# NTT123/vietTTS

Hardware: NVIDIA H100
Metric: audio_samples_per_sec (higher is better)
Workload: dtype f32 (bf16x3 split products on wgmma tensor cores, fp32 accumulate/storage)

## Files before the change

### viettts_b200/csrc/api.cu

```cuda
#include <stdarg.h>

#include <algorithm>

#include <dlfcn.h>

#include "stream_common.cuh"

std::string g_vtts_create_error;

int vtts_ctx::fail(int code, const char* fmt, ...) {
  char buf[1024];
  va_list ap;
  va_start(ap, fmt);
  vsnprintf(buf, sizeof(buf), fmt, ap);
  va_end(ap);
  err = buf;
  return code;
}

int vtts_ctx::ensure_ws(size_t bytes) {
  vtts_ctx* ctx = this;
  if (bytes <= ws_bytes) return VTTS_OK;
  clear_taps();
  if (ws) {
// ... 253 lines not shown
int vtts_create(int device, vtts_ctx** out) {
  if (!out) {
    g_vtts_create_error = "vtts_create: out is NULL";
    return VTTS_ERR_BAD_ARG;
  }
  *out = nullptr;
  int n = 0;
  cudaError_t e = cudaGetDeviceCount(&n);
  if (e != cudaSuccess || n == 0) {
    g_vtts_create_error = std::string("vtts_create: no CUDA device (") + cudaGetErrorString(e) + "); there is no CPU fallback";
    cudaGetLastError();
    return VTTS_ERR_NO_DEVICE;
  }
  if (device < 0 || device >= n) {
    g_vtts_create_error = "vtts_create: device index out of range";
    return VTTS_ERR_BAD_ARG;
  }
  cudaDeviceProp prop;
  if ((e = cudaSetDevice(device)) != cudaSuccess || (e = cudaGetDeviceProperties(&prop, device)) != cudaSuccess) {
    g_vtts_create_error = std::string("vtts_create: ") + cudaGetErrorString(e);
    return VTTS_ERR_CUDA;
  }
  if (prop.major != 9 || prop.minor != 0) {
    char buf[256];
    snprintf(buf, sizeof(buf), "vtts_create: device %d is sm_%d%d; this library contains sm_90a code only", device, prop.major, prop.minor);
    g_vtts_create_error = buf;
    return VTTS_ERR_NO_DEVICE;
  }
  vtts_ctx* ctx = new vtts_ctx();
  ctx->device = device;
  ctx->sm_count = prop.multiProcessorCount;
  ctx->cc_major = prop.major;
  ctx->cc_minor = prop.minor;
  ctx->hbm_bytes = prop.totalGlobalMem;
  if ((e = cudaStreamCreateWithFlags(&ctx->own_stream, cudaStreamNonBlocking)) != cudaSuccess) {
    g_vtts_create_error = std::string("vtts_create: ") + cudaGetErrorString(e);
    delete ctx;
    return VTTS_ERR_CUDA;
  }
  for (int i = 0; i < vtts_ctx::NSTAGE; ++i) {
    cudaEventCreate(&ctx->ev0[i]);
    cudaEventCreate(&ctx->ev1[i]);
  }
  if ((e = cudaEventCreateWithFlags(&ctx->tail, cudaEventDisableTiming)) != cudaSuccess) {
    g_vtts_create_error = std::string("vtts_create: ") + cudaGetErrorString(e);
    delete ctx;
    return VTTS_ERR_CUDA;
  }
  if (cudaMalloc(&ctx->d_err, sizeof(int)) != cudaSuccess || cudaMemset(ctx->d_err, 0, sizeof(int)) != cudaSuccess) {
    g_vtts_create_error = "vtts_create: cannot allocate the error flag";
    delete ctx;
    return VTTS_ERR_CUDA;
  }
  if (cudaMalloc(&ctx->d_tc_sched, 2 * sizeof(int)) != cudaSuccess || cudaMemset(ctx->d_tc_sched, 0, 2 * sizeof(int)) != cudaSuccess) {
    g_vtts_create_error = "vtts_create: cannot allocate the tile scheduler counters";
    delete ctx;
    return VTTS_ERR_CUDA;
  }
  if (cudaMalloc(&ctx->d_tc_dbg, 256 * 16 * sizeof(long long)) != cudaSuccess) {
    g_vtts_create_error = "vtts_create: cannot allocate the profiling counters";
    delete ctx;
    return VTTS_ERR_CUDA;
  }
  cudaMemset(ctx->d_tc_dbg, 0, 256 * 16 * sizeof(long long));
  *out = ctx;
  return VTTS_OK;
}

int vtts_destroy(vtts_ctx* ctx) {
  if (!ctx) return VTTS_OK;
  cudaSetDevice(ctx->device);
  cudaDeviceSynchronize();
  for (auto& m : kModels) vtts_free_weights(ctx->*m.w);
  vtts_resample_free(ctx);
  cudaFree(ctx->mel_fb); cudaFree(ctx->mel_lo); cudaFree(ctx->mel_hi); cudaFree(ctx->fft_tw); cudaFree(ctx->hann);
  cudaFree(ctx->ws); cudaFree(ctx->dstage); cudaFree(ctx->d_err); cudaFree(ctx->d_tc_sched); cudaFree(ctx->d_tc_dbg);
  if (ctx->hpin) cudaFreeHost(ctx->hpin);
  for (int i = 0; i < vtts_ctx::NSTAGE; ++i) {
    cudaEventDestroy(ctx->ev0[i]);
    cudaEventDestroy(ctx->ev1[i]);
  }
  if (ctx->tail) cudaEventDestroy(ctx->tail);
  if (ctx->own_stream) cudaStreamDestroy(ctx->own_stream);
  delete ctx;
  return VTTS_OK;
}

const char* vtts_last_error(vtts_ctx* ctx) { return ctx ? ctx->err.c_str() : g_vtts_create_error.c_str(); }

int vtts_device_info(vtts_ctx* ctx, int* sm_count, int* cc_major, int* cc_minor, int64_t* hbm_bytes) {
  if (!ctx) return VTTS_ERR_BAD_ARG;
  if (sm_count) *sm_count = ctx->sm_count;
  if (cc_major) *cc_major = ctx->cc_major;
  if (cc_minor) *cc_minor = ctx->cc_minor;
  if (hbm_bytes) *hbm_bytes = (int64_t)ctx->hbm_bytes;
  return VTTS_OK;
}

int vtts_set_precision(vtts_ctx* ctx, int mode) {
  if (!ctx) return VTTS_ERR_BAD_ARG;
  if (mode != VTTS_PRECISION_FP32 && mode != VTTS_PRECISION_BF16X3 && mode != VTTS_PRECISION_FP16)
    return ctx->fail(VTTS_ERR_BAD_ARG, "set_precision: mode %d", mode);
  ctx->precision = mode;
  return VTTS_OK;
}

int vtts_get_precision(vtts_ctx* ctx) { return ctx ? ctx->precision : VTTS_ERR_BAD_ARG; }
// ... 556 lines not shown
```

### viettts_b200/csrc/tc_conv.cu

```cuda
#include <cuda_bf16.h>

#include <algorithm>

#include "tc_common.cuh"
#include "vtts_internal.cuh"

namespace {

using namespace tcx;

constexpr int NCWG = 2;
constexpr int NCONS = NCWG * 128;
constexpr int PROD_WARP = NCONS / 32;
constexpr int NCONV = 96;
constexpr int NTHREADS = NCONS + 32 + NCONV;
constexpr int NA = 4;
constexpr int HALO = 64;
constexpr int PAIR_OVERLAP = 16;
constexpr int NQ = 2;
constexpr int NREADERS = (NCONS + NCONV) / 32;

constexpr int SUB_CG = 4;
constexpr int SUB_HALO = 1;
constexpr int SUB_RS = NCWG * 64 + SUB_HALO;
constexpr int SUB_CSB = SUB_RS * 64 + 32;
constexpr int SUB_STAGE = SUB_CG * SUB_CSB;
static_assert(SUB_RS * 4 % 32 == 4 && SUB_CSB / 4 % 32 == 24, "bank-conflict-free converter stores");

template <int N, int MW, int PAIRF, bool STAGED = false, bool SUB = false>
struct TcCfg {
  static constexpr int R = 64 * MW * NCWG;
  static constexpr int R_OUT = R - PAIR_OVERLAP;
  static constexpr int RA = R + HALO;
  static constexpr int A_STAGE = RA * 64;
  static constexpr int NAS = SUB ? (N == 64 ? 4 : 2) : NA;
  static constexpr int A_BYTES = SUB ? NAS * SUB_STAGE : NA * A_STAGE;
  static constexpr int W_STAGE = N * 64;
  static constexpr int NW = N == 256 ? 4 : 8;
  static constexpr int NCH2 = PAIRF ? N / 16 : 0;
  static constexpr int EPI_NC = N < 128 ? N : 128;
  static constexpr int EPI_LD = EPI_NC + 8;
  static constexpr int EPI_WG = 64 * EPI_LD + N;
  static constexpr int EPI_STAGE = STAGED ? NCWG * EPI_WG * 4 : 0;
  static constexpr int SMEM_BYTES =
      A_BYTES + NW * W_STAGE + NCH2 * A_STAGE + EPI_STAGE + (2 * NA + 2 * NW + 2 * NQ) * 8 + NQ * 4 + 1024;
  static_assert(SMEM_BYTES <= 227 * 1024, "shared memory of one CTA");
};

struct Ring {
  uint32_t s = 0, p = 0;
  template <int NS>
  __device__ __forceinline__ void next() { if (++s == NS) { s = 0; p ^= 1; } }
};

struct Tile {
  int pi, b, tt;
};
__device__ __forceinline__ Tile decode_tile(int t, int nprob, int tiles_per_row) {
  Tile d;
  d.pi = t % nprob; t /= nprob;
  d.tt = t % tiles_per_row;
  d.b = t / tiles_per_row;
  return d;
}

__device__ __forceinline__ int take_ticket(int* sched, int ntiles) {
  const int t = (int)gridDim.x + atomicAdd(&sched[0], 1);
  if (t < ntiles) return t;
  __threadfence();
  if (atomicAdd(&sched[1], 1) == (int)gridDim.x - 1) {
    atomicExch(&sched[0], 0);
    atomicExch(&sched[1], 0);
  }
  return -1;
}

struct TileQueue {
  int* id;
  uint64_t* full;
  uint64_t* empty;
  Ring r;
  __device__ __forceinline__ void put(int t, int* err, long long& acc) {
    mbar_wait_t(&empty[r.s], r.p ^ 1, err, 6, acc);
    id[r.s] = t;
    mbar_arrive(&full[r.s]);
    r.next<NQ>();
  }
  __device__ __forceinline__ int get(int* err, long long& acc) {
    int t = 0;
    if ((threadIdx.x & 31) == 0) {
      mbar_wait_t(&full[r.s], r.p, err, 6, acc);
      t = id[r.s];
      mbar_arrive(&empty[r.s]);
    }
    r.next<NQ>();
    return __shfl_sync(0xffffffffu, t, 0);
  }
};

__device__ __forceinline__ float div3_rn(float s) {
  constexpr float y = 0x1.555556p-2f;
  const float q0 = __fmul_rn(s, y);
  const float q1 = __fmaf_rn(__fmaf_rn(-q0, 3.0f, s), y, q0);
  return (s == 0.f || fabsf(s) == __int_as_float(0x7f800000)) ? s : q1;
}

template <int QN, int RS, int CSB, bool F16, bool LOADS_FIRST = false>
__device__ __forceinline__ void convert_rows(uint8_t* stage, int ct, const float* x0, const float* x1, const float* x2, int ld, int ch0,
                                             int row_base, int rows, int lo, int valid, int pre_mode, float slope) {
  static_assert(NCONV % QN == 0, "whole rows per converter step");
  constexpr int RSTEP = NCONV / QN, RA = RS;
  const int q = ct % QN;
  const int r0 = ct / QN;
  uint8_t* st = stage + (q >> 2) * CSB + (((q >> 1) & 1) * RA) * 16 + (q & 1) * 8;
  const int coff = ch0 + q * 4;
  constexpr int U = 8;
  for (int rr0 = r0; rr0 < rows; rr0 += RSTEP * U) {
    float4 v[U];
    if constexpr (LOADS_FIRST) {
      float4 a[U], bb[U];
      bool in[U];
#pragma unroll
      for (int u = 0; u < U; ++u) {
        const int rr = rr0 + u * RSTEP;
        const int t = row_base + rr;
        in[u] = rr < rows && t >= lo && t < valid;
        v[u] = a[u] = bb[u] = make_float4(0.f, 0.f, 0.f, 0.f);
        if (in[u]) {
// ... 101 lines not shown
        const int lane = threadIdx.x & 31, wl = (threadIdx.x >> 5) & 3;
        uint32_t fa_hi[MW][4], fa_lo[MW][4];
#pragma unroll
        for (int mt = 0; mt < MW; ++mt) {
          const int row = (wg * MW + mt) * 64 + wl * 16 + ((lane >> 3) & 1) * 8 + (lane & 7) + j * dil;
          const uint32_t addr = a_base + ((lane >> 4) * RA + row) * 16;
          ldmatrix_x4(fa_hi[mt], addr);
          ldmatrix_x4(fa_lo[mt], addr + 2 * RA * 16);
        }
        wgmma_fence();
#pragma unroll
        for (int mt = 0; mt < MW; ++mt) {
          wgmma_rs<N>(acc[mt], fa_hi[mt], b_hi, first);
          wgmma_rs<N>(acc[mt], fa_hi[mt], b_lo, 1u);
          wgmma_rs<N>(acc[mt], fa_lo[mt], b_hi, 1u);
        }
        wgmma_commit();
        wgmma_wait<0>();
        if (lane == 0) mbar_arrive(&w_empty[rw.s]);
        rw.next<NW>();
        continue;
      }
      wgmma_fence();
#pragma unroll
      for (int mt = 0; mt < MW; ++mt) {
        const uint32_t row = a_base + ((wg * MW + mt) * 64 + j * dil) * 16;
        const uint64_t a_hi = a_tmpl | (uint64_t)(row >> 4);
        const uint64_t a_lo = a_tmpl | (uint64_t)((row + 2 * RA * 16) >> 4);
        if constexpr (F16) {
          wgmma<N, true>(acc[mt], a_hi, b_hi, first);
        } else {
          wgmma<N>(acc[mt], a_hi, b_hi, first);
          wgmma<N>(acc[mt], a_hi, b_lo, 1u);
          wgmma<N>(acc[mt], a_lo, b_hi, 1u);
        }
      }
      wgmma_commit();
      wgmma_wait<1>();
      if (lane0) {
        if (pend_w >= 0) mbar_arrive(&w_empty[pend_w]);
        if (pend_a >= 0) mbar_arrive(&a_empty[pend_a]);
      }
      pend_w = (int)rw.s;
      pend_a = (A_FROM_RING && j == k - 1) ? (int)ra.s : -1;
      rw.next<NW>();
    }
    if constexpr (A_FROM_RING) ra.next<NA>();
  }
  wgmma_wait<0>();
  if (lane0) {
    if (pend_w >= 0) mbar_arrive(&w_empty[pend_w]);
    if (pend_a >= 0) mbar_arrive(&a_empty[pend_a]);
  }
}

template <int N, int NW, int NAS, bool F16>
__device__ __forceinline__ void consume_rows(float (&acc)[N / 2], int wg, uint32_t a_st_u32, uint64_t* a_full, uint64_t* a_empty, Ring& ra,
                                             uint32_t w_st_u32, uint64_t* w_full, uint64_t* w_empty, Ring& rw, int nch, int k, int dil,
                                             int* err, long long& w_a, long long& w_w) {
  const uint64_t a_tmpl = make_desc(0, SUB_RS * 16, 128);
  const uint64_t b_tmpl = make_desc(0, (F16 ? 1 : 2) * N * 16, 128);
  const bool lane0 = (threadIdx.x & 31) == 0;
  int pend_w = -1, pend_a = -1;
  for (int c0 = 0; c0 < nch; c0 += SUB_CG) {
    mbar_wait_t(&a_full[ra.s], ra.p, err, 2, w_a);
    const uint32_t a_blk = a_st_u32 + ra.s * SUB_STAGE + wg * 64 * 16;
    for (int cl = 0; cl < SUB_CG; ++cl) {
      for (int j = 0; j < k; ++j) {
        mbar_wait_t(&w_full[rw.s], rw.p, err, 3, w_w);
        const uint32_t w_base = w_st_u32 + rw.s * (N * 64);
        const uint64_t b_hi = b_tmpl | (uint64_t)(w_base >> 4);
        const uint64_t b_lo = b_tmpl | (uint64_t)((w_base + N * 16) >> 4);
        const uint32_t first = ((c0 + cl) | j) != 0 ? 1u : 0u;
        const uint32_t row = a_blk + cl * SUB_CSB + j * dil * 16;
        const uint64_t a_hi = a_tmpl | (uint64_t)(row >> 4);
        const uint64_t a_lo = a_tmpl | (uint64_t)((row + 2 * SUB_RS * 16) >> 4);
        wgmma_fence();
        if constexpr (F16) {
          wgmma<N, true>(acc, a_hi, b_hi, first);
        } else {
          wgmma<N>(acc, a_hi, b_hi, first);
          wgmma<N>(acc, a_hi, b_lo, 1u);
          wgmma<N>(acc, a_lo, b_hi, 1u);
        }
        wgmma_commit();
        wgmma_wait<1>();
        if (lane0) {
          if (pend_w >= 0) mbar_arrive(&w_empty[pend_w]);
          if (pend_a >= 0) mbar_arrive(&a_empty[pend_a]);
        }
        pend_w = (int)rw.s;
        pend_a = (cl == SUB_CG - 1 && j == k - 1) ? (int)ra.s : -1;
        rw.next<NW>();
      }
    }
    ra.next<NAS>();
  }
  wgmma_wait<0>();
  if (lane0) {
    if (pend_w >= 0) mbar_arrive(&w_empty[pend_w]);
    if (pend_a >= 0) mbar_arrive(&a_empty[pend_a]);
  }
}

__device__ __forceinline__ void cp_async16(void* smem_dst, const void* gsrc) {
  asm volatile("cp.async.cg.shared.global [%0], [%1], 16;" ::"r"(smem_u32(smem_dst)), "l"(gsrc) : "memory");
}
__device__ __forceinline__ void cp_async_commit() { asm volatile("cp.async.commit_group;" ::: "memory"); }
__device__ __forceinline__ void cp_async_wait_all() { asm volatile("cp.async.wait_all;" ::: "memory"); }

__device__ __forceinline__ void init_barriers(uint64_t* bars, int nw) {
  uint64_t* a_full = bars;
  uint64_t* a_empty = bars + NA;
  uint64_t* w_full = bars + 2 * NA;
  uint64_t* w_empty = bars + 2 * NA + nw;
  uint64_t* q_full = bars + 2 * NA + 2 * nw;
  uint64_t* q_empty = q_full + NQ;
  for (int i = 0; i < NA; ++i) { mbar_init(&a_full[i], NCONV); mbar_init(&a_empty[i], NCONS / 32); }
  for (int i = 0; i < nw; ++i) { mbar_init(&w_full[i], 1); mbar_init(&w_empty[i], NCONS / 32); }
  for (int i = 0; i < NQ; ++i) { mbar_init(&q_full[i], 1); mbar_init(&q_empty[i], NREADERS); }
  asm volatile("fence.mbarrier_init.release.cluster;" ::: "memory");
}

__device__ __forceinline__ TileQueue tile_queue(uint64_t* bars, int nw) {
  uint64_t* q_full = bars + 2 * NA + 2 * nw;
  return TileQueue{reinterpret_cast<int*>(q_full + 2 * NQ), q_full, q_full + NQ, Ring{}};
}

__device__ __forceinline__ int sub_elem(const TcLaunch& L, const TcProb& P, int tau, int col) {
  return (tau * P.out_stride + P.out_off) * L.out_ld + P.out_e0 + col;
}

#define PRODUCER_TILES                                                                     \
  TileQueue q = tile_queue(bars, NW);                                                      \
  long long w_q = 0;                                                                       \
  int t_next = blockIdx.x;                                                                 \
  q.put(t_next, L.err, w_q);                                                               \
  auto next_tile = [&]() {                                                                 \
    const int t = t_next;                                                                  \
    if (t >= 0) { t_next = take_ticket(L.sched, L.ntiles); q.put(t_next, L.err, w_q); }    \
    return t;                                                                              \
  };
#define READER_TILES                                                                       \
  TileQueue q = tile_queue(bars, NW);                                                      \
  long long w_q = 0;                                                                       \
  auto next_tile = [&]() { return q.get(L.err, w_q); };

template <int N, int EPI, int MW, bool F16, bool SUB>
__global__ void __launch_bounds__(NTHREADS, 1) tc_conv_kernel(const __grid_constant__ TcLaunch L) {
  static_assert(!SUB || EPI == 0, "sub-row output uses the plain epilogue");
  using Cfg = TcCfg<N, MW, 0, EPI == 0, SUB>;
  constexpr int R = Cfg::R, RA = Cfg::RA, NW = Cfg::NW, NAS = Cfg::NAS;
  extern __shared__ uint8_t smem_raw[];
  uint8_t* smem = (uint8_t*)(((uintptr_t)smem_raw + 1023) & ~(uintptr_t)1023);
  uint8_t* a_st = smem;
  uint8_t* w_st = smem + Cfg::A_BYTES;
  float* epi_st = reinterpret_cast<float*>(smem_raw + (w_st + NW * Cfg::W_STAGE - smem_raw));
  uint64_t* bars = reinterpret_cast<uint64_t*>(w_st + NW * Cfg::W_STAGE + Cfg::EPI_STAGE);
  uint64_t* a_full = bars;
  uint64_t* a_empty = bars + NA;
  uint64_t* w_full = bars + 2 * NA;
  uint64_t* w_empty = bars + 2 * NA + NW;

  const int tid = threadIdx.x;
  const int warp = __shfl_sync(0xffffffffu, tid >> 5, 0);
  if (tid == 0) init_barriers(bars, NW);
  __syncthreads();

  const int nch = L.Cin / 16;

  constexpr bool ROW_BOUNDS = EPI == 0;
#define TILE_LOOP_BEGIN                                                           \
  for (int tile; (tile = next_tile()) >= 0;) {                                    \
    const Tile td = decode_tile(tile, L.nprob, L.tiles_per_row);                   \
    const int b = td.b;                                                            \
    const int tau0 = td.tt * R;                                                    \
    const TcProb& P = L.p[td.pi];                                                  \
    int valid = L.T_rows, in_lo = 0, out_hi = 0;                                  \
    if (ROW_BOUNDS && P.rb) {                                                     \
      in_lo = P.rb[3 * b]; valid = P.rb[3 * b + 1]; out_hi = P.rb[3 * b + 2];     \
      if (!SUB && tau0 * P.out_stride + P.out_off >= out_hi) continue;            \
    } else {                                                                      \
      if (L.len) {                                                                \
        const int v = L.len[b] * L.len_mul;                                       \
        valid = v < valid ? v : valid;                                            \
      }                                                                           \
      if (!SUB && tau0 >= valid) continue;                                        \
    }                                                                             \
    const int e_lim = SUB ? (P.rb ? out_hi * L.out_sub : valid * L.out_ld) : 0;   \
    if (SUB && sub_elem(L, P, tau0, 0) >= e_lim) continue;
#define TILE_LOOP_END }

  if (warp == PROD_WARP) {
    if ((tid & 31) == 0) {
      Ring rw;
      long long w_e = 0;
      PRODUCER_TILES
      TILE_LOOP_BEGIN
        (void)b; (void)tau0; (void)in_lo; (void)valid; (void)out_hi; (void)e_lim;
        for (int mt = 0; mt < (SUB ? MW : 1); ++mt) produce_weights<N, NW, F16>(w_st, w_full, w_empty, rw, P.wpk, nch, P.k, L.err, w_e);
      TILE_LOOP_END
      if (L.dbg) L.dbg[(size_t)blockIdx.x * 16 + 4] = w_e;
    }
  } else if (warp > PROD_WARP) {
    const int ct = tid - NCONS - 32;
    Ring ra;
    long long w_ae = 0;
    READER_TILES
    TILE_LOOP_BEGIN
      const int k = P.k, dil = P.dil;
      const size_t in_base = (size_t)b * L.T_rows * L.in_ld;
      const float* x1 = L.pre_mode == 2 ? P.x1 + in_base : nullptr;
      const float* x2 = L.pre_mode == 2 ? P.x2 + in_base : nullptr;
      if constexpr (SUB) {
        for (int mt = 0; mt < MW; ++mt)
          for (int c0 = 0; c0 < nch; c0 += SUB_CG) {
            mbar_wait_t(&a_empty[ra.s], ra.p ^ 1, L.err, 5, w_ae);
            convert_rows<SUB_CG * 4, SUB_RS, SUB_CSB, F16, true>(a_st + ra.s * SUB_STAGE, ct, P.x0 + in_base, x1, x2, L.in_ld, c0 * 16,
                                                            tau0 + P.in_off + mt * NCWG * 64, NCWG * 64 + (k - 1) * dil, in_lo, valid,
                                                            L.pre_mode, L.pre_slope);
            fence_proxy_async();
            mbar_arrive(&a_full[ra.s]);
            ra.next<NAS>();
          }
      } else {
        for (int c = 0; c < nch; ++c) {
          mbar_wait_t(&a_empty[ra.s], ra.p ^ 1, L.err, 5, w_ae);
          convert_chunk<RA, F16>(a_st + ra.s * Cfg::A_STAGE, ct, P.x0 + in_base, x1, x2, L.in_ld, c, tau0 + P.in_off, R + (k - 1) * dil,
                            in_lo, valid, L.pre_mode, L.pre_slope);
          fence_proxy_async();
          mbar_arrive(&a_full[ra.s]);
          ra.next<NA>();
        }
      }
      (void)out_hi; (void)e_lim;
    TILE_LOOP_END
    if (L.dbg && ct == 0) L.dbg[(size_t)blockIdx.x * 16 + 5] = w_ae;
  } else {
    const int wg = warp >> 2, lane = tid & 31;
    float acc[MW][N / 2];
    Ring ra, rw;
    long long w_a = 0, w_w = 0, t_epi = 0;
    const long long t_begin = clock64();
    const int n_valid = (EPI && L.n_valid > 0) ? L.n_valid : N;
    const int post_act = EPI ? L.post_act : 0;
    constexpr int EPI_NC = Cfg::EPI_NC, EPI_LD = Cfg::EPI_LD, RPS = 128 / (EPI_NC / 4), NQ4 = 64 / RPS;
    float* stg = epi_st + wg * Cfg::EPI_WG;
    float* stg_bias = stg + 64 * EPI_LD;
    const int fr = (warp & 3) * 16 + (lane >> 2), fc = 2 * (lane & 3);
    const int dr = (tid & 127) / (EPI_NC / 4), dq = (tid & 127) % (EPI_NC / 4);
// ... 65 lines not shown
#pragma unroll
            for (int i = 0; i < NQ4; ++i) {
              const int row = i * RPS + dr, tau = blk + row;
              const int e = (tau * ostride + ooff) * L.out_ld + oe0 + nh * EPI_NC + dq * 4;
              if (elem_ok(tau, e))
                *reinterpret_cast<float4*>(P.out + out_base + e) = *reinterpret_cast<const float4*>(stg + row * EPI_LD + dq * 4);
            }
            named_bar(2 + wg, 128);
          }
        }
      } else {
        const int row_w = tau0 + wg * MW * 64 + (warp & 3) * 16 + (lane >> 2);
#pragma unroll
        for (int mt = 0; mt < MW; ++mt)
#pragma unroll
          for (int h = 0; h < 2; ++h) {
            const int tau = row_w + mt * 64 + 8 * h;
            if (!row_ok(tau)) continue;
            const size_t orow = out_base + (size_t)(tau * ostride + ooff) * L.out_ld;
#pragma unroll
            for (int jn = 0; jn < N / 8; ++jn) {
              const int col = jn * 8 + 2 * (lane & 3);
              if (col >= n_valid) continue;
              float2 o = make_float2(acc[mt][jn * 4 + 2 * h], acc[mt][jn * 4 + 2 * h + 1]);
              const float2 bi = __ldg(reinterpret_cast<const float2*>(P.bias + col));
              o.x += bi.x; o.y += bi.y;
              if (P.bn_mean) {
                const float2 mu = __ldg(reinterpret_cast<const float2*>(P.bn_mean + col));
                const float2 iv = __ldg(reinterpret_cast<const float2*>(P.bn_inv + col));
                const float2 of = __ldg(reinterpret_cast<const float2*>(P.bn_off + col));
                o.x = (o.x - mu.x) * iv.x + of.x; o.y = (o.y - mu.y) * iv.y + of.y;
              }
              if (post_act == 1) { o.x = tanhf(o.x); o.y = tanhf(o.y); }
              else if (post_act == 2) { o.x = fmaxf(o.x, 0.f); o.y = fmaxf(o.y, 0.f); }
              if (P.resid) {
                const float2 r = __ldg(reinterpret_cast<const float2*>(P.resid + orow + col));
                o.x += r.x; o.y += r.y;
              }
              *reinterpret_cast<float2*>(P.out + orow + col) = o;
            }
          }
      }
      t_epi += clock64() - t_epi0;
    TILE_LOOP_END
    if (L.dbg && tid == 0) {
      long long* d = L.dbg + (size_t)blockIdx.x * 16;
      d[0] = clock64() - t_begin; d[1] = t_epi; d[2] = w_a; d[3] = w_w;
    }
  }
#undef TILE_LOOP_BEGIN
#undef TILE_LOOP_END
}

template <int N, int MW, bool A2_REGS, bool F16>
__global__ void __launch_bounds__(NTHREADS, 1) tc_pair_kernel(const __grid_constant__ TcPairLaunch L) {
  using Cfg = TcCfg<N, MW, 1>;
  constexpr int R = Cfg::R, R_OUT = Cfg::R_OUT, RA = Cfg::RA, NW = Cfg::NW, NCH = N / 16;
  extern __shared__ uint8_t smem_raw[];
  uint8_t* smem = (uint8_t*)(((uintptr_t)smem_raw + 1023) & ~(uintptr_t)1023);
  uint8_t* a_st = smem;
  uint8_t* w_st = smem + NA * Cfg::A_STAGE;
  uint8_t* mid = w_st + NW * Cfg::W_STAGE;
  uint64_t* bars = reinterpret_cast<uint64_t*>(mid + Cfg::NCH2 * Cfg::A_STAGE);
  uint64_t* a_full = bars;
  uint64_t* a_empty = bars + NA;
  uint64_t* w_full = bars + 2 * NA;
  uint64_t* w_empty = bars + 2 * NA + NW;

  const int tid = threadIdx.x;
  const int warp = __shfl_sync(0xffffffffu, tid >> 5, 0);
  if (tid == 0) init_barriers(bars, NW);
  __syncthreads();

#define TILE_LOOP_BEGIN                                                   \
  for (int tile; (tile = next_tile()) >= 0;) {                            \
    const Tile td = decode_tile(tile, L.nprob, L.tiles_per_row);        \
    const int b = td.b;                                                    \
    const int tau0 = td.tt * R_OUT;                                        \
    int valid = L.T_rows;                                                 \
    if (L.len) {                                                          \
      const int v = L.len[b] * L.len_mul;                                 \
      valid = v < valid ? v : valid;                                      \
    }                                                                     \
    if (tau0 >= valid) continue;                                          \
    const TcPairProb& P = L.p[td.pi];                                      \
    const int k = P.k, dil = P.dil, h2 = (k - 1) / 2;
#define TILE_LOOP_END }

  if (warp == PROD_WARP) {
    if ((tid & 31) == 0) {
      Ring rw;
      long long w_e = 0;
      PRODUCER_TILES
      TILE_LOOP_BEGIN
        (void)b; (void)tau0; (void)dil; (void)h2;
        produce_weights<N, NW, F16>(w_st, w_full, w_empty, rw, P.w1pk, NCH, k, L.err, w_e);
        produce_weights<N, NW, F16>(w_st, w_full, w_empty, rw, P.w2pk, NCH, k, L.err, w_e);
      TILE_LOOP_END
    }
  } else if (warp > PROD_WARP) {
    const int ct = tid - NCONS - 32;
    Ring ra;
    long long w_ae = 0;
    READER_TILES
    TILE_LOOP_BEGIN
      const float* x = P.x + (size_t)b * L.T_rows * N;
      const int row_base = tau0 - h2 - (k - 1) * dil / 2;
      for (int c = 0; c < NCH; ++c) {
        mbar_wait_t(&a_empty[ra.s], ra.p ^ 1, L.err, 5, w_ae);
        convert_chunk<RA, F16>(a_st + ra.s * Cfg::A_STAGE, ct, x, nullptr, nullptr, N, c, row_base, R + (k - 1) * dil, 0, valid, 1, L.slope);
        fence_proxy_async();
        mbar_arrive(&a_full[ra.s]);
        ra.next<NA>();
      }
    TILE_LOOP_END
  } else {
    const int wg = warp >> 2, lane = tid & 31;
    float acc[MW][N / 2];
    Ring ra, rw;
    long long w_a = 0, w_w = 0;
    const long long t_begin = clock64();
    const float slope = L.slope;
    READER_TILES
    TILE_LOOP_BEGIN
      consume<N, MW, RA, NW, true, false, F16>(acc, wg, smem_u32(a_st), a_full, a_empty, ra, smem_u32(w_st), w_full, w_empty, rw, NCH, k, dil,
                                               L.err, w_a, w_w);
      const int lr_w = wg * MW * 64 + (warp & 3) * 16 + (lane >> 2);
#pragma unroll
      for (int mt = 0; mt < MW; ++mt)
#pragma unroll
        for (int h = 0; h < 2; ++h) {
          const int lr = lr_w + mt * 64 + 8 * h;
          const int u = tau0 - h2 + lr;
          const bool inside = u >= 0 && u < valid;
#pragma unroll
          for (int jn = 0; jn < N / 8; ++jn) {
            const int col = jn * 8 + 2 * (lane & 3);
            const float2 bi = __ldg(reinterpret_cast<const float2*>(P.b1 + col));
            const float v0 = inside ? lrelu(acc[mt][jn * 4 + 2 * h] + bi.x, slope) : 0.f;
            const float v1 = inside ? lrelu(acc[mt][jn * 4 + 2 * h + 1] + bi.y, slope) : 0.f;
            uint8_t* dst = mid + (col >> 4) * Cfg::A_STAGE + (((col >> 3) & 1) * RA + lr) * 16 + (col & 7) * 2;
            if constexpr (F16) {
              *reinterpret_cast<uint32_t*>(dst) = f16x2_sat(v0, v1);
            } else {
              const __nv_bfloat162 hi = __floats2bfloat162_rn(v0, v1);
              const __nv_bfloat162 lo = __floats2bfloat162_rn(v0 - __low2float(hi), v1 - __high2float(hi));
              *reinterpret_cast<__nv_bfloat162*>(dst) = hi;
              *reinterpret_cast<__nv_bfloat162*>(dst + 2 * RA * 16) = lo;
            }
          }
        }
      fence_proxy_async();
      named_bar(1, NCONS);
      consume<N, MW, RA, NW, false, A2_REGS, F16>(acc, wg, smem_u32(mid), a_full, a_empty, ra, smem_u32(w_st), w_full, w_empty, rw, NCH, k, 1,
                                                  L.err, w_a, w_w);
      named_bar(1, NCONS);
      const float* x = P.x + (size_t)b * L.T_rows * N;
      float* out = P.out + (size_t)b * L.T_rows * N;
#pragma unroll
      for (int mt = 0; mt < MW; ++mt)
#pragma unroll
        for (int h = 0; h < 2; ++h) {
          const int lr = lr_w + mt * 64 + 8 * h;
          const int tau = tau0 + lr;
          if (lr >= R_OUT || tau >= valid) continue;
#pragma unroll
          for (int jn = 0; jn < N / 8; ++jn) {
            const int col = jn * 8 + 2 * (lane & 3);
            const float2 bi = __ldg(reinterpret_cast<const float2*>(P.b2 + col));
            const float2 r = __ldg(reinterpret_cast<const float2*>(x + (size_t)tau * N + col));
            float2 o;
            o.x = acc[mt][jn * 4 + 2 * h] + bi.x + r.x;
            o.y = acc[mt][jn * 4 + 2 * h + 1] + bi.y + r.y;
            *reinterpret_cast<float2*>(out + (size_t)tau * N + col) = o;
          }
        }
    TILE_LOOP_END
    if (L.dbg && tid == 0) {
      long long* d = L.dbg + (size_t)blockIdx.x * 16;
      d[0] = clock64() - t_begin; d[2] = w_a; d[3] = w_w;
    }
  }
#undef TILE_LOOP_BEGIN
#undef TILE_LOOP_END
}

template <bool F16>
__global__ void pack_w_kernel(const float* __restrict__ w, uint16_t* __restrict__ dst, int k, int Cin, int Cout_total, int n0, int N) {
  const size_t total = (size_t)k * Cin * N;
  for (size_t idx = blockIdx.x * (size_t)blockDim.x + threadIdx.x; idx < total; idx += (size_t)gridDim.x * blockDim.x) {
    const int n = idx % N;
    const int i = (idx / N) % Cin;
    const int j = idx / ((size_t)N * Cin);
    const float v = (n0 + n) < Cout_total ? w[((size_t)j * Cin + i) * Cout_total + n0 + n] : 0.f;
    const int c = i / 16, kh = (i % 16) / 8, e = i % 8;
    if constexpr (F16) {
      const size_t blk = ((size_t)c * k + j) * (size_t)(2 * N * 8);
      dst[blk + ((size_t)kh * N + n) * 8 + e] = (uint16_t)(f16x2_sat(v, 0.f) & 0xffffu);
      continue;
    }
    const __nv_bfloat16 hi = __float2bfloat16_rn(v);
    const __nv_bfloat16 lo = __float2bfloat16_rn(v - __bfloat162float(hi));
    const size_t blk = ((size_t)c * k + j) * (size_t)(4 * N * 8);
    dst[blk + ((size_t)(kh * 2 + 0) * N + n) * 8 + e] = __bfloat16_as_ushort(hi);
    dst[blk + ((size_t)(kh * 2 + 1) * N + n) * 8 + e] = __bfloat16_as_ushort(lo);
  }
}

template <int N, int EPI, int MW, bool F16, bool SUB = false>
int launch_cfg(vtts_ctx* ctx, TcLaunch& L, cudaStream_t st) {
  using Cfg = TcCfg<N, MW, 0, EPI == 0, SUB>;
  static bool attr_done_dev[64] = {};
  if (!attr_done_dev[ctx->device & 63]) {
    VTTS_CUDA(cudaFuncSetAttribute(tc_conv_kernel<N, EPI, MW, F16, SUB>, cudaFuncAttributeMaxDynamicSharedMemorySize, Cfg::SMEM_BYTES));
    attr_done_dev[ctx->device & 63] = true;
  }
  for (int i = 0; i < L.nprob; ++i)
    if ((L.p[i].k - 1) * L.p[i].dil > (SUB ? SUB_HALO : HALO)) return ctx->fail(VTTS_ERR_BAD_ARG, "tc_conv: halo too large");
  if (SUB && L.Cin % (SUB_CG * 16)) return ctx->fail(VTTS_ERR_BAD_ARG, "tc_conv: sub-row output needs Cin %% %d == 0, not %d", SUB_CG * 16, L.Cin);
  std::stable_sort(L.p, L.p + L.nprob, [](const TcProb& a, const TcProb& b) { return a.k > b.k; });
  L.tiles_per_row = ((L.tile_rows > 0 ? L.tile_rows : L.T_rows) + Cfg::R - 1) / Cfg::R;
  L.ntiles = L.nprob * L.tiles_per_row * L.B;
  const int grid = L.ntiles < ctx->sm_count ? L.ntiles : ctx->sm_count;
  tc_conv_kernel<N, EPI, MW, F16, SUB><<<grid, NTHREADS, Cfg::SMEM_BYTES, st>>>(L);
  ctx->launches++;
  VTTS_CUDA(cudaGetLastError());
  return VTTS_OK;
}

template <int N>
int launch_n(vtts_ctx* ctx, TcLaunch& L, cudaStream_t st) {
  constexpr int MW = N >= 256 ? 1 : (N == 128 ? 2 : 4);
  bool generic = L.post_act != 0 || (L.n_valid > 0 && L.n_valid < N);
  bool rb = false;
  for (int i = 0; i < L.nprob; ++i) {
    generic |= L.p[i].bn_mean != nullptr;
    rb |= L.p[i].rb != nullptr;
  }
  if ((rb || L.out_sub) && generic) return ctx->fail(VTTS_ERR_BAD_ARG, "tc_conv: per-row bounds and sub-row output use the plain epilogue");
  if (L.out_sub < 0 || (L.out_sub && (L.out_sub % 4 || L.out_ld % L.out_sub)))
    return ctx->fail(VTTS_ERR_BAD_ARG, "tc_conv: output rows of %d floats in tile rows of %d", L.out_sub, L.out_ld);
  if (!generic) {
    const int row_w = L.out_sub ? L.out_sub : L.out_ld;
    if ((int64_t)L.rows_out * row_w > INT32_MAX) return ctx->fail(VTTS_ERR_BAD_ARG, "tc_conv: %d output rows of %d", L.rows_out, row_w);
    bool aligned = L.out_ld % 4 == 0;
    for (int i = 0; i < L.nprob; ++i) aligned &= (((uintptr_t)L.p[i].out | (uintptr_t)L.p[i].resid | (uintptr_t)L.p[i].bias) & 15) == 0;
    if (!aligned) return ctx->fail(VTTS_ERR_BAD_ARG, "tc_conv: the plain epilogue needs 16-byte aligned out / resid rows and bias (out_ld %d)", L.out_ld);
  }
  if (L.f16 && generic) return ctx->fail(VTTS_ERR_BAD_ARG, "tc_conv: fp16 operands use the plain epilogue");
  if (L.f16) return L.out_sub ? launch_cfg<N, 0, MW, true, true>(ctx, L, st) : launch_cfg<N, 0, MW, true>(ctx, L, st);
  if (generic) return launch_cfg<N, 1, MW, false>(ctx, L, st);
  return L.out_sub ? launch_cfg<N, 0, MW, false, true>(ctx, L, st) : launch_cfg<N, 0, MW, false>(ctx, L, st);
}

template <int N, int MW, bool A2_REGS, bool F16 = false>
int launch_pair(vtts_ctx* ctx, TcPairLaunch& L, cudaStream_t st) {
  using Cfg = TcCfg<N, MW, 1>;
  static bool attr_done_dev[64] = {};
  if (!attr_done_dev[ctx->device & 63]) {
    VTTS_CUDA(cudaFuncSetAttribute(tc_pair_kernel<N, MW, A2_REGS, F16>, cudaFuncAttributeMaxDynamicSharedMemorySize, Cfg::SMEM_BYTES));
    attr_done_dev[ctx->device & 63] = true;
  }
  for (int i = 0; i < L.nprob; ++i)
    if (L.p[i].k - 1 > PAIR_OVERLAP || (L.p[i].k - 1) * L.p[i].dil > HALO) return ctx->fail(VTTS_ERR_BAD_ARG, "tc_pair: halo too large");
  std::stable_sort(L.p, L.p + L.nprob, [](const TcPairProb& a, const TcPairProb& b) { return a.k > b.k; });
  L.tiles_per_row = (L.T_rows + Cfg::R_OUT - 1) / Cfg::R_OUT;
  L.ntiles = L.nprob * L.tiles_per_row * L.B;
  const int grid = L.ntiles < ctx->sm_count ? L.ntiles : ctx->sm_count;
  tc_pair_kernel<N, MW, A2_REGS, F16><<<grid, NTHREADS, Cfg::SMEM_BYTES, st>>>(L);
  ctx->launches++;
  VTTS_CUDA(cudaGetLastError());
  return VTTS_OK;
}

}

size_t vtts_tc_packed_elems(int k, int Cin, int N, bool f16) { return (size_t)k * Cin * N * (f16 ? 1 : 2); }

int vtts_tc_pack_weights(vtts_ctx* ctx, const float* w, void* dst, int k, int Cin, int Cout_total, int n0, int N, bool f16) {
  if (f16) pack_w_kernel<true><<<256, 256>>>(w, reinterpret_cast<uint16_t*>(dst), k, Cin, Cout_total, n0, N);
  else pack_w_kernel<false><<<256, 256>>>(w, reinterpret_cast<uint16_t*>(dst), k, Cin, Cout_total, n0, N);
  VTTS_CUDA(cudaGetLastError());
  return VTTS_OK;
}

int vtts_tc_tile_n(int Cout) { return Cout <= 32 ? 32 : (Cout <= 64 ? 64 : (Cout <= 128 ? 128 : 256)); }

size_t vtts_tc_conv_packed_bytes(int k, int Cin, int Cout, bool f16) {
  const int N = vtts_tc_tile_n(Cout), nt = (Cout + N - 1) / N;
  return ((vtts_tc_packed_elems(k, Cin, N, f16) * 2 + 255) & ~size_t(255)) * nt;
}

int vtts_tc_pack_conv(vtts_ctx* ctx, const float* w, int k, int Cin, int Cout, bool f16, char*& cursor, std::vector<void*>& out) {
  const int N = vtts_tc_tile_n(Cout), nt = (Cout + N - 1) / N;
  for (int t = 0; t < nt; ++t) {
    int rc = vtts_tc_pack_weights(ctx, w, cursor, k, Cin, Cout, t * N, N, f16);
    if (rc) return rc;
    out.push_back(cursor);
    cursor += (vtts_tc_packed_elems(k, Cin, N, f16) * 2 + 255) & ~size_t(255);
  }
  return VTTS_OK;
}

int vtts_conv_dispatch(vtts_ctx* ctx, const ConvLaunch& L, void* const* wpk, cudaStream_t st) {
  if (ctx->precision == VTTS_PRECISION_FP32 || wpk == nullptr) return vtts_launch_conv(ctx, L, st);
  const int N = vtts_tc_tile_n(L.Cout), nt = (L.Cout + N - 1) / N;
  TcLaunch TL;
  auto reset = [&]() {
    memset(&TL, 0, sizeof(TL));
    TL.Cin = L.Cin; TL.N = N; TL.in_ld = L.Cin; TL.out_ld = L.Cout; TL.B = L.B; TL.T_rows = L.T_rows; TL.rows_out = L.rows_out;
    TL.len = L.len; TL.len_mul = L.len_mul; TL.pre_mode = L.pre_mode; TL.pre_slope = L.pre_slope; TL.post_act = L.post_act;
    TL.n_valid = (L.Cout % N) ? (L.Cout % N) : N;
  };
  reset();
  for (int pass = 0; pass < 2; ++pass) {
    const bool partial = pass == 1;
    if (partial && (L.Cout % N) == 0) break;
    reset();
    TL.n_valid = partial ? (L.Cout % N) : N;
    for (int pi = 0; pi < L.nprob; ++pi) {
      const ConvProb& cp = L.p[pi];
// ... 63 lines not shown
```

### viettts_b200/csrc/vtts_internal.cuh

```cuda
#pragma once
#include <cuda_runtime.h>
#include <stdint.h>
#include <stdio.h>
#include <string.h>
#include <algorithm>
#include <string>
#include <vector>

#include "../../include/viettts_b200.h"

namespace vc {
constexpr int MEL = 80;
constexpr int HOP = 256;
constexpr int NFFT = 1024;
constexpr int NBINS = 513;
constexpr int ENC_D = 256;
constexpr int ENC_OUT = 512;
constexpr int DEC_H = 512;
constexpr int PRENET = 256;
constexpr int POSTNET = 512;
constexpr int VOCAB = 256;
constexpr int SIL_INDEX = 0;
constexpr int WORD_END_INDEX = 3;
constexpr int LAUNCH_ROWS = 128;
// ... 50 lines not shown
  const void* wpk;
  const float* bias;
  const float* resid;
  const float* bn_mean;
  const float* bn_inv;
  const float* bn_off;
  float* out;
  int k, dil, in_off, out_stride, out_off;
  int out_e0;
  const int* rb;
};

struct TcLaunch {
  TcProb p[8];
  int nprob;
  int Cin, N;
  int in_ld, out_ld;
  int B, T_rows, rows_out;
  const int* len;
  int len_mul;
  int pre_mode;
  float pre_slope;
  int out_sub;
  int post_act;
  int n_valid;
  int f16;
  int tile_rows;
  int tiles_per_row, ntiles;
  int* sched;
  int* err;
  long long* dbg;
};

struct TcPairProb {
  const float* x;
  const void* w1pk;
  const void* w2pk;
  const float* b1;
  const float* b2;
  float* out;
  int k, dil;
};

struct TcPairLaunch {
  TcPairProb p[3];
  int nprob;
  int N;
  int B, T_rows;
  const int* len;
  int len_mul;
  float slope;
  int f16;
  int tiles_per_row, ntiles;
  int* sched;
  int* err;
  long long* dbg;
};

struct ModelWeights {
  float* blob = nullptr;
  std::vector<float*> t;
  float* derived = nullptr;
  std::vector<float*> d;
  void* wpk = nullptr;
  std::vector<void*> wpk_t;
  std::vector<int> tile0;
  bool loaded = false;
  void* const* tiles(int conv) const { return &wpk_t[tile0[conv]]; }
};

struct vtts_ctx {
  int device = 0;
  int precision = 1;
  int* d_err = nullptr;
  int* d_tc_sched = nullptr;
  long long* d_tc_dbg = nullptr;
  bool tc_dbg_on = false;
  int fuse_pairs = 1;
  int pair_ts = 2;
  int sm_count = 0;
  int cc_major = 0, cc_minor = 0;
  size_t hbm_bytes = 0;
  std::string err;
  int64_t launches = 0;
  cudaStream_t own_stream = nullptr;
  cudaEvent_t tail = nullptr;
  int order_depth = 0;

  ModelWeights hg;
  ModelWeights ac;
  ModelWeights du;

  float* mel_fb = nullptr;
  int* mel_lo = nullptr;
  int* mel_hi = nullptr;
  float* fft_tw = nullptr;
  float* hann = nullptr;
  bool fft_ready = false;
  bool mel_loaded = false;

  void* ws = nullptr;
  size_t ws_bytes = 0;
  void* hpin = nullptr;
  size_t hpin_bytes = 0;
  void* dstage = nullptr;
  size_t dstage_bytes = 0;
// ... 233 lines not shown
```

Measured before the change: 57.47 million.

## Keep C=32 resblock pair weights resident in shared memory with per-problem CTA affinity

For the N=32, MW=2 pair kernel, both convolutions' packed weights are bulk-copied into shared memory once per problem instead of being streamed through the weight ring for every tile. A new affine tile scheduler splits CTAs across problems in proportion to kernel size, so each CTA mostly stays on one problem and rarely reloads weights; it work-steals from other problems when its own runs out. The residual input is also prefetched into registers before the MMAs to hide its load latency. The cost is extra shared memory and register pressure, a more complex scheduler with four counters, and a limit of kernel size 11 on this path.

```diff
diff --git a/viettts_b200/csrc/api.cu b/viettts_b200/csrc/api.cu
--- a/viettts_b200/csrc/api.cu
+++ b/viettts_b200/csrc/api.cu
@@ -329,7 +329,7 @@
     delete ctx;
     return VTTS_ERR_CUDA;
   }
-  if (cudaMalloc(&ctx->d_tc_sched, 2 * sizeof(int)) != cudaSuccess || cudaMemset(ctx->d_tc_sched, 0, 2 * sizeof(int)) != cudaSuccess) {
+  if (cudaMalloc(&ctx->d_tc_sched, 4 * sizeof(int)) != cudaSuccess || cudaMemset(ctx->d_tc_sched, 0, 4 * sizeof(int)) != cudaSuccess) {
     g_vtts_create_error = "vtts_create: cannot allocate the tile scheduler counters";
     delete ctx;
     return VTTS_ERR_CUDA;
diff --git a/viettts_b200/csrc/tc_conv.cu b/viettts_b200/csrc/tc_conv.cu
--- a/viettts_b200/csrc/tc_conv.cu
+++ b/viettts_b200/csrc/tc_conv.cu
@@ -1,6 +1,7 @@
 #include <cuda_bf16.h>
 
 #include <algorithm>
+#include <type_traits>
 
 #include "tc_common.cuh"
 #include "vtts_internal.cuh"
@@ -27,7 +28,9 @@
 constexpr int SUB_STAGE = SUB_CG * SUB_CSB;
 static_assert(SUB_RS * 4 % 32 == 4 && SUB_CSB / 4 % 32 == 24, "bank-conflict-free converter stores");
 
-template <int N, int MW, int PAIRF, bool STAGED = false, bool SUB = false>
+constexpr int RES_KMAX = 11;
+
+template <int N, int MW, int PAIRF, bool STAGED = false, bool SUB = false, bool F16 = false>
 struct TcCfg {
   static constexpr int R = 64 * MW * NCWG;
   static constexpr int R_OUT = R - PAIR_OVERLAP;
@@ -36,15 +39,20 @@
   static constexpr int NAS = SUB ? (N == 64 ? 4 : 2) : NA;
   static constexpr int A_BYTES = SUB ? NAS * SUB_STAGE : NA * A_STAGE;
   static constexpr int W_STAGE = N * 64;
-  static constexpr int NW = N == 256 ? 4 : 8;
+  static constexpr bool W_RES = PAIRF == 2;
+  static constexpr int W_BLK = F16 ? N * 32 : N * 64;
+  static constexpr int W_CONV = N / 16 * RES_KMAX * W_BLK;
+  static constexpr int NW = W_RES ? 1 : (N == 256 ? 4 : 8);
+  static constexpr int W_BYTES = W_RES ? 2 * W_CONV : NW * W_STAGE;
   static constexpr int NCH2 = PAIRF ? N / 16 : 0;
   static constexpr int EPI_NC = N < 128 ? N : 128;
   static constexpr int EPI_LD = EPI_NC + 8;
   static constexpr int EPI_WG = 64 * EPI_LD + N;
   static constexpr int EPI_STAGE = STAGED ? NCWG * EPI_WG * 4 : 0;
   static constexpr int SMEM_BYTES =
-      A_BYTES + NW * W_STAGE + NCH2 * A_STAGE + EPI_STAGE + (2 * NA + 2 * NW + 2 * NQ) * 8 + NQ * 4 + 1024;
+      A_BYTES + W_BYTES + NCH2 * A_STAGE + EPI_STAGE + (2 * NA + 2 * NW + 2 * NQ) * 8 + NQ * 4 + 1024;
   static_assert(SMEM_BYTES <= 227 * 1024, "shared memory of one CTA");
+  static_assert(!W_RES || (N == 32 && MW == 2), "resident weights: the C = 32 pair in 256-row tiles");
 };
 
 struct Ring {
@@ -74,6 +82,48 @@
   }
   return -1;
 }
+
+struct LinearSched {
+  int* sched;
+  int ntiles;
+  template <class Launch>
+  __device__ __forceinline__ explicit LinearSched(const Launch& L) : sched(L.sched), ntiles(L.ntiles) {}
+  __device__ __forceinline__ int first() const { return (int)blockIdx.x; }
+  __device__ __forceinline__ int next() { return take_ticket(sched, ntiles); }
+};
+
+constexpr int SCHED_DONE = 3;
+struct AffineSched {
+  int* sched;
+  const int* cta0;
+  int nprob, ptiles, p;
+  __device__ __forceinline__ explicit AffineSched(const TcPairLaunch& L)
+      : sched(L.sched), cta0(L.cta0), nprob(L.nprob), ptiles(L.ntiles / L.nprob), p(0) {
+    for (int q = 1; q < nprob; ++q)
+      if ((int)blockIdx.x >= cta0[q]) p = q;
+  }
+  __device__ __forceinline__ int n(int q) const { return cta0[q + 1] - cta0[q]; }
+  __device__ __forceinline__ int first() {
+    const int l = (int)blockIdx.x - cta0[p];
+    return l < ptiles ? l * nprob + p : next();
+  }
+  __device__ __forceinline__ int next() {
+    for (;;) {
+      const int t = n(p) + atomicAdd(&sched[p], 1);
+      if (t < ptiles) return t * nprob + p;
+      int most = 0;
+      for (int q = 0; q < nprob; ++q) {
+        const int left = ptiles - n(q) - *(volatile int*)&sched[q];
+        if (left > most) { most = left; p = q; }
+      }
+      if (most == 0) break;
+    }
+    __threadfence();
+    if (atomicAdd(&sched[SCHED_DONE], 1) == (int)gridDim.x - 1)
+      for (int q = 0; q <= SCHED_DONE; ++q) atomicExch(&sched[q], 0);
+    return -1;
+  }
+};
 
 struct TileQueue {
   int* id;
@@ -281,6 +331,54 @@
     if (pend_w >= 0) mbar_arrive(&w_empty[pend_w]);
     if (pend_a >= 0) mbar_arrive(&a_empty[pend_a]);
   }
+}
+
+template <int N, int MW, int RA, bool A_FROM_RING, bool F16>
+__device__ __forceinline__ void consume_resident(float (&acc)[MW][N / 2], int wg, uint32_t a_st_u32, uint64_t* a_full, uint64_t* a_empty,
+                                                 Ring& ra, uint32_t w_st_u32, int nch, int k, int dil, int* err, long long& w_a) {
+  constexpr int WB = F16 ? N * 32 : N * 64;
+  const uint64_t a_tmpl = make_desc(0, RA * 16, 128);
+  const uint64_t b_tmpl = make_desc(0, (F16 ? 1 : 2) * N * 16, 128);
+  const bool lane0 = (threadIdx.x & 31) == 0;
+  int pend_a = -1;
+  for (int c = 0; c < nch; ++c) {
+    uint32_t a_base;
+    if constexpr (A_FROM_RING) {
+      mbar_wait_t(&a_full[ra.s], ra.p, err, 2, w_a);
+      a_base = a_st_u32 + ra.s * (RA * 64);
+    } else {
+      a_base = a_st_u32 + c * (RA * 64);
+    }
+    wgmma_fence();
+    for (int j = 0; j < k; ++j) {
+      const uint32_t w_base = w_st_u32 + (c * k + j) * WB;
+      const uint64_t b_hi = b_tmpl | (uint64_t)(w_base >> 4);
+      const uint64_t b_lo = b_tmpl | (uint64_t)((w_base + N * 16) >> 4);
+      const uint32_t first = (c | j) != 0 ? 1u : 0u;
+#pragma unroll
+      for (int mt = 0; mt < MW; ++mt) {
+        const uint32_t row = a_base + ((wg * MW + mt) * 64 + j * dil) * 16;
+        const uint64_t a_hi = a_tmpl | (uint64_t)(row >> 4);
+        const uint64_t a_lo = a_tmpl | (uint64_t)((row + 2 * RA * 16) >> 4);
+        if constexpr (F16) {
+          wgmma<N, true>(acc[mt], a_hi, b_hi, first);
+        } else {
+          wgmma<N>(acc[mt], a_hi, b_hi, first);
+          wgmma<N>(acc[mt], a_hi, b_lo, 1u);
+          wgmma<N>(acc[mt], a_lo, b_hi, 1u);
+        }
+      }
+    }
+    wgmma_commit();
+    if constexpr (A_FROM_RING) {
+      wgmma_wait<1>();
+      if (lane0 && pend_a >= 0) mbar_arrive(&a_empty[pend_a]);
+      pend_a = (int)ra.s;
+      ra.next<NA>();
+    }
+  }
+  wgmma_wait<0>();
+  if (lane0 && pend_a >= 0) mbar_arrive(&a_empty[pend_a]);
 }
 
 template <int N, int NW, int NAS, bool F16>
@@ -360,14 +458,15 @@
   return (tau * P.out_stride + P.out_off) * L.out_ld + P.out_e0 + col;
 }
 
-#define PRODUCER_TILES                                                                     \
+#define PRODUCER_TILES(SCHED)                                                              \
   TileQueue q = tile_queue(bars, NW);                                                      \
   long long w_q = 0;                                                                       \
-  int t_next = blockIdx.x;                                                                 \
+  SCHED sch(L);                                                                            \
+  int t_next = sch.first();                                                                \
   q.put(t_next, L.err, w_q);                                                               \
   auto next_tile = [&]() {                                                                 \
     const int t = t_next;                                                                  \
-    if (t >= 0) { t_next = take_ticket(L.sched, L.ntiles); q.put(t_next, L.err, w_q); }    \
+    if (t >= 0) { t_next = sch.next(); q.put(t_next, L.err, w_q); }                        \
     return t;                                                                              \
   };
 #define READER_TILES                                                                       \
@@ -424,7 +523,7 @@
     if ((tid & 31) == 0) {
       Ring rw;
       long long w_e = 0;
-      PRODUCER_TILES
+      PRODUCER_TILES(LinearSched)
       TILE_LOOP_BEGIN
         (void)b; (void)tau0; (void)in_lo; (void)valid; (void)out_hi; (void)e_lim;
         for (int mt = 0; mt < (SUB ? MW : 1); ++mt) produce_weights<N, NW, F16>(w_st, w_full, w_empty, rw, P.wpk, nch, P.k, L.err, w_e);
@@ -596,15 +695,19 @@
 #undef TILE_LOOP_END
 }
 
+template <int N, int MW, bool A2_REGS>
+constexpr int pair_cfg() { return N == 32 && MW == 2 && !A2_REGS ? 2 : 1; }
+
 template <int N, int MW, bool A2_REGS, bool F16>
 __global__ void __launch_bounds__(NTHREADS, 1) tc_pair_kernel(const __grid_constant__ TcPairLaunch L) {
-  using Cfg = TcCfg<N, MW, 1>;
+  using Cfg = TcCfg<N, MW, pair_cfg<N, MW, A2_REGS>(), false, false, F16>;
   constexpr int R = Cfg::R, R_OUT = Cfg::R_OUT, RA = Cfg::RA, NW = Cfg::NW, NCH = N / 16;
+  constexpr bool W_RES = Cfg::W_RES;
   extern __shared__ uint8_t smem_raw[];
   uint8_t* smem = (uint8_t*)(((uintptr_t)smem_raw + 1023) & ~(uintptr_t)1023);
   uint8_t* a_st = smem;
   uint8_t* w_st = smem + NA * Cfg::A_STAGE;
-  uint8_t* mid = w_st + NW * Cfg::W_STAGE;
+  uint8_t* mid = w_st + Cfg::W_BYTES;
   uint64_t* bars = reinterpret_cast<uint64_t*>(mid + Cfg::NCH2 * Cfg::A_STAGE);
   uint64_t* a_full = bars;
   uint64_t* a_empty = bars + NA;
@@ -635,11 +738,25 @@
     if ((tid & 31) == 0) {
       Ring rw;
       long long w_e = 0;
-      PRODUCER_TILES
+      int loaded = -1;
+      uint32_t pe = 0;
+      using Sched = std::conditional_t<W_RES, AffineSched, LinearSched>;
+      PRODUCER_TILES(Sched)
       TILE_LOOP_BEGIN
         (void)b; (void)tau0; (void)dil; (void)h2;
-        produce_weights<N, NW, F16>(w_st, w_full, w_empty, rw, P.w1pk, NCH, k, L.err, w_e);
-        produce_weights<N, NW, F16>(w_st, w_full, w_empty, rw, P.w2pk, NCH, k, L.err, w_e);
+        if constexpr (W_RES) {
+          if (td.pi != loaded) {
+            if (loaded >= 0) { mbar_wait_t(&w_empty[0], pe, L.err, 4, w_e); pe ^= 1; }
+            const uint32_t bytes = NCH * k * Cfg::W_BLK;
+            mbar_expect_tx(&w_full[0], 2 * bytes);
+            bulk_g2s(w_st, P.w1pk, bytes, &w_full[0]);
+            bulk_g2s(w_st + Cfg::W_CONV, P.w2pk, bytes, &w_full[0]);
+            loaded = td.pi;
+          }
+        } else {
+          produce_weights<N, NW, F16>(w_st, w_full, w_empty, rw, P.w1pk, NCH, k, L.err, w_e);
+          produce_weights<N, NW, F16>(w_st, w_full, w_empty, rw, P.w2pk, NCH, k, L.err, w_e);
+        }
       TILE_LOOP_END
     }
   } else if (warp > PROD_WARP) {
@@ -665,10 +782,36 @@
     long long w_a = 0, w_w = 0;
     const long long t_begin = clock64();
     const float slope = L.slope;
+    uint32_t res = 0;
     READER_TILES
     TILE_LOOP_BEGIN
-      consume<N, MW, RA, NW, true, false, F16>(acc, wg, smem_u32(a_st), a_full, a_empty, ra, smem_u32(w_st), w_full, w_empty, rw, NCH, k, dil,
-                                               L.err, w_a, w_w);
+      if constexpr (W_RES) {
+        if ((res >> 1) != (uint32_t)td.pi + 1) {
+          if (res > 1 && lane == 0) mbar_arrive(&w_empty[0]);
+          mbar_wait_t(&w_full[0], res & 1, L.err, 3, w_w);
+          res = ((uint32_t)td.pi + 1) << 1 | ((res & 1) ^ 1);
+        }
+      }
+      float2 xr[MW][2][N / 8];
+      if constexpr (W_RES) {
+        const float* xb = P.x + (size_t)b * L.T_rows * N;
+#pragma unroll
+        for (int mt = 0; mt < MW; ++mt)
+#pragma unroll
+          for (int h = 0; h < 2; ++h) {
+            const int lr = wg * MW * 64 + (warp & 3) * 16 + (lane >> 2) + mt * 64 + 8 * h;
+            const int tau = tau0 + lr;
+            const bool ok = lr < R_OUT && tau < valid;
+#pragma unroll
+            for (int jn = 0; jn < N / 8; ++jn)
+              xr[mt][h][jn] = ok ? __ldg(reinterpret_cast<const float2*>(xb + (size_t)tau * N + jn * 8 + 2 * (lane & 3))) : make_float2(0.f, 0.f);
+          }
+      }
+      if constexpr (W_RES)
+        consume_resident<N, MW, RA, true, F16>(acc, wg, smem_u32(a_st), a_full, a_empty, ra, smem_u32(w_st), NCH, k, dil, L.err, w_a);
+      else
+        consume<N, MW, RA, NW, true, false, F16>(acc, wg, smem_u32(a_st), a_full, a_empty, ra, smem_u32(w_st), w_full, w_empty, rw, NCH, k,
+                                                 dil, L.err, w_a, w_w);
       const int lr_w = wg * MW * 64 + (warp & 3) * 16 + (lane >> 2);
 #pragma unroll
       for (int mt = 0; mt < MW; ++mt)
@@ -696,8 +839,11 @@
         }
       fence_proxy_async();
       named_bar(1, NCONS);
-      consume<N, MW, RA, NW, false, A2_REGS, F16>(acc, wg, smem_u32(mid), a_full, a_empty, ra, smem_u32(w_st), w_full, w_empty, rw, NCH, k, 1,
-                                                  L.err, w_a, w_w);
+      if constexpr (W_RES)
+        consume_resident<N, MW, RA, false, F16>(acc, wg, smem_u32(mid), a_full, a_empty, ra, smem_u32(w_st) + Cfg::W_CONV, NCH, k, 1, L.err, w_a);
+      else
+        consume<N, MW, RA, NW, false, A2_REGS, F16>(acc, wg, smem_u32(mid), a_full, a_empty, ra, smem_u32(w_st), w_full, w_empty, rw, NCH, k, 1,
+                                                    L.err, w_a, w_w);
       named_bar(1, NCONS);
       const float* x = P.x + (size_t)b * L.T_rows * N;
       float* out = P.out + (size_t)b * L.T_rows * N;
@@ -712,7 +858,7 @@
           for (int jn = 0; jn < N / 8; ++jn) {
             const int col = jn * 8 + 2 * (lane & 3);
             const float2 bi = __ldg(reinterpret_cast<const float2*>(P.b2 + col));
-            const float2 r = __ldg(reinterpret_cast<const float2*>(x + (size_t)tau * N + col));
+            const float2 r = W_RES ? xr[mt][h][jn] : __ldg(reinterpret_cast<const float2*>(x + (size_t)tau * N + col));
             float2 o;
             o.x = acc[mt][jn * 4 + 2 * h] + bi.x + r.x;
             o.y = acc[mt][jn * 4 + 2 * h + 1] + bi.y + r.y;
@@ -799,7 +945,7 @@
 
 template <int N, int MW, bool A2_REGS, bool F16 = false>
 int launch_pair(vtts_ctx* ctx, TcPairLaunch& L, cudaStream_t st) {
-  using Cfg = TcCfg<N, MW, 1>;
+  using Cfg = TcCfg<N, MW, pair_cfg<N, MW, A2_REGS>(), false, false, F16>;
   static bool attr_done_dev[64] = {};
   if (!attr_done_dev[ctx->device & 63]) {
     VTTS_CUDA(cudaFuncSetAttribute(tc_pair_kernel<N, MW, A2_REGS, F16>, cudaFuncAttributeMaxDynamicSharedMemorySize, Cfg::SMEM_BYTES));
@@ -811,6 +957,18 @@
   L.tiles_per_row = (L.T_rows + Cfg::R_OUT - 1) / Cfg::R_OUT;
   L.ntiles = L.nprob * L.tiles_per_row * L.B;
   const int grid = L.ntiles < ctx->sm_count ? L.ntiles : ctx->sm_count;
+  if (Cfg::W_RES) {
+    int ksum = 0, kcum = 0;
+    for (int i = 0; i < L.nprob; ++i) {
+      if (L.p[i].k > RES_KMAX) return ctx->fail(VTTS_ERR_BAD_ARG, "tc_pair: C = %d holds pairs of k <= %d in shared memory, not %d", N, RES_KMAX, L.p[i].k);
+      ksum += L.p[i].k;
+    }
+    for (int i = 0; i < L.nprob; ++i) {
+      L.cta0[i] = (int)(((int64_t)2 * grid * kcum + ksum) / (2 * ksum));
+      kcum += L.p[i].k;
+    }
+    L.cta0[L.nprob] = grid;
+  }
   tc_pair_kernel<N, MW, A2_REGS, F16><<<grid, NTHREADS, Cfg::SMEM_BYTES, st>>>(L);
   ctx->launches++;
   VTTS_CUDA(cudaGetLastError());
diff --git a/viettts_b200/csrc/vtts_internal.cuh b/viettts_b200/csrc/vtts_internal.cuh
--- a/viettts_b200/csrc/vtts_internal.cuh
+++ b/viettts_b200/csrc/vtts_internal.cuh
@@ -126,6 +126,7 @@
   float slope;
   int f16;
   int tiles_per_row, ntiles;
+  int cta0[4];
   int* sched;
   int* err;
   long long* dbg;
```

Result: no change. 57.82 million, median of 6 (+0.6%).
